# greysun/GraphEmbeddings

Hardware: AMD Instinct MI355X
Metric: scored triples/sec/GPU (d=200) (higher is better)
Workload: dtype f32

## Files before the change

### graphembeddings_amd/csrc/ge_prep.h

```cpp
#pragma once
#include "ge_common.h"

namespace ge {

constexpr int kSlotDirect = -2;
constexpr int kPrepThreads = 1024;
constexpr int kPrepWaves = kPrepThreads / kWave;
constexpr int kItemCap = 16;
constexpr int64_t kSub = 4096;
constexpr int kMaxRadix = 256;
constexpr unsigned long long kInvalidKey = ~0ull;

__host__ __device__ inline int64_t step_row(int64_t first_row, int64_t T, int64_t B, int64_t s) {
  int64_t first = first_row % T;
  if (first + B > T) first = 0;
  const int64_t n0 = (T - first) / B;
  if (s < n0) return first + s * B;
  const int64_t per = T / B;
  return ((s - n0) % per) * B;
}

struct PrepLayout {
  int64_t B, negs, units, n_sub, S, P, off_slot, off_order, off_sub, sub_stride, off_items, off_islots, stride;
  int epu;
};
__host__ __device__ inline PrepLayout prep_layout(int64_t B, int64_t negs = 0) {
  PrepLayout L;
  L.B = B;
  L.negs = negs;
  L.epu = negs > 0 ? 3 : 4;
  L.units = negs > 0 ? (1 + negs) * B : B;
  L.n_sub = (L.units + kSub - 1) / kSub;
  const int64_t s = L.units < kSub ? L.units : kSub;
  const int64_t gran = negs > 0 ? 1024 : 256;
  L.S = (s + gran - 1) / gran * gran;
  L.P = L.epu * L.S;
  L.off_slot = 3 * B;
  L.off_order = (negs == 0 && L.n_sub > 1) ? 9 * B : -1;
  L.off_sub = negs > 0 ? (3 * negs * B + 63) / 64 * 64 : ((L.off_order >= 0 ? 10 : 9) * B + 63) / 64 * 64;
  L.off_items = 64;
  L.off_islots = 64 + 2 * L.P;
  L.sub_stride = 64 + 2 * L.P + kItemCap * L.P;
  L.stride = L.off_sub + L.n_sub * L.sub_stride;
  return L;
}

struct TileGeom {
  int P, n_sub;
  int64_t stride;
  int64_t off_slot;
  int64_t off_sub, sub_stride;
  int off_items, off_islots;
};
inline TileGeom geom_of(const PrepLayout& L) {
  return TileGeom{(int)L.P, (int)L.n_sub, L.stride, L.off_slot, L.off_sub, L.sub_stride, (int)L.off_items, (int)L.off_islots};
}
inline TileGeom geom_plain(int P, int n_sub) {
  const int64_t sub = 64 + 2 * (int64_t)P + kItemCap * (int64_t)P;
  return TileGeom{P, n_sub, n_sub * sub, -1, 0, sub, 64, 64 + 2 * P};
}

struct ShardOut {
  int32_t R;
  int64_t B;
  int32_t* pos_src;
  int32_t* neg_src;
  int32_t* req_row;
  const int32_t* tile_heads;
  int32_t peer;
};

struct SortBits { int n_pass, bits; };
inline SortBits sort_bits_for(int64_t N) {
  int nbits = 1;
  while (((int64_t)1 << nbits) <= N) ++nbits;
  SortBits s;
  s.n_pass = (nbits + 7) / 8;
  s.bits = (nbits + s.n_pass - 1) / s.n_pass;
  if (s.bits < 6) s.bits = 6;
  return s;
}

__device__ __forceinline__ int wave_incl_add(int v, int lane) {
#pragma unroll
  for (int o = 1; o < kWave; o <<= 1) { const int t = __shfl_up(v, o, kWave); if (lane >= o) v += t; }
  return v;
}
__device__ __forceinline__ int wave_incl_max(int v, int lane) {
#pragma unroll
  for (int o = 1; o < kWave; o <<= 1) { const int t = __shfl_up(v, o, kWave); if (lane >= o) v = max(v, t); }
  return v;
}

struct StepSource {
  const int32_t* pos; int64_t B; const int32_t* id_to_type; int64_t N; const int64_t* type_offsets;
  int32_t n_types; const int32_t* type_ids; uint64_t seed, step; int32_t padded_size, mode, negs;
};

__device__ __forceinline__ void unit_keys(const StepSource& S, int64_t j, bool batch_heads, int32_t* __restrict__ neg,
                                          unsigned long long (&k)[4]) {
  if (S.negs > 0) {
    const int64_t B = S.B;
    const int64_t i = j < B ? j : (j - B) % B;
    int32_t t3[3] = {S.pos[3 * i], S.pos[3 * i + 1], S.pos[3 * i + 2]};
    if (j >= B) {
      const int64_t kk = (j - B) / B;
      const uint64_t stepk = S.step * (uint64_t)S.negs + (uint64_t)kk;
      const bool heads_k = (S.mode == GE_CORRUPT_BATCH_COIN) ? batch_coin_heads(S.seed, stepk) : false;
      int col;
      const int32_t repl = corrupt_one(t3, i, heads_k, S.id_to_type, S.N, S.type_offsets, S.n_types, S.type_ids, S.seed,
                                       stepk, S.padded_size, S.mode, col);
      t3[col] = repl;
      int32_t* o = neg + 3 * (kk * B + i);
      o[0] = t3[0]; o[1] = t3[1]; o[2] = t3[2];
    }
    const bool bad = t3[0] < 0 || t3[1] < 0 || t3[2] < 0 || t3[0] >= S.N || t3[1] >= S.N || t3[2] >= S.N;
#pragma unroll
    for (int X = 0; X < 3; ++X)
      k[X] = bad ? kInvalidKey : (((unsigned long long)(uint32_t)t3[X] << 32) | (uint32_t)(3 * j + X));
    k[3] = kInvalidKey;
    return;
  }
  const int64_t i = j;
  int32_t p[3] = {S.pos[3 * i], S.pos[3 * i + 1], S.pos[3 * i + 2]};
  int col;
  const int32_t repl = corrupt_one(p, i, batch_heads, S.id_to_type, S.N, S.type_offsets, S.n_types, S.type_ids, S.seed,
                                   S.step, S.padded_size, S.mode, col);
  int32_t n[3] = {p[0], p[1], p[2]};
  n[col] = repl;
  neg[3 * i] = n[0]; neg[3 * i + 1] = n[1]; neg[3 * i + 2] = n[2];
  const bool bad = p[0] < 0 || p[1] < 0 || p[2] < 0 || p[0] >= S.N || p[1] >= S.N || p[2] >= S.N || repl < 0 || repl >= S.N;
#pragma unroll
  for (int X = 0; X < 3; ++X)
    k[X] = bad ? kInvalidKey : (((unsigned long long)(uint32_t)p[X] << 32) | (uint32_t)(6 * i + X));
  k[3] = (bad || repl == p[col]) ? kInvalidKey : (((unsigned long long)(uint32_t)repl << 32) | (uint32_t)(6 * i + 3 + col));
}

}
```

### graphembeddings_amd/csrc/ge_train.hip

```cpp
#include "ge_prep.h"
#include "ge_launch.h"
#include <cmath>

namespace ge {

__global__ __launch_bounds__(kPrepThreads) void train_prepare_kernel(
    const int32_t* __restrict__ triples, int64_t T, int64_t first_row, int64_t B, int64_t s0,
    const int32_t* __restrict__ id_to_type, int64_t N, const int64_t* __restrict__ type_offsets,
    int32_t n_types, const int32_t* __restrict__ type_ids, uint64_t seed, uint64_t global_step0,
    int32_t padded_size, int32_t mode, int direct, int n_pass, int bits, int negs, int32_t* __restrict__ prep) {
  extern __shared__ __attribute__((aligned(16))) unsigned long long keys[];
  const PrepLayout L = prep_layout(B, negs);
  const int P = (int)L.P, R = P / kPrepThreads;
  unsigned* hist = reinterpret_cast<unsigned*>(keys + P);
  int* wtot = reinterpret_cast<int*>(hist + kPrepWaves * kMaxRadix);
  const int tid = threadIdx.x, lane = tid & (kWave - 1), wave = tid >> 6;
  const int sub = blockIdx.y;
  const int64_t s = s0 + blockIdx.x;
  const int32_t* pos = triples + 3 * step_row(first_row, T, B, s);
  int32_t* rec = prep + (int64_t)blockIdx.x * L.stride;
  int32_t* neg = rec;
  int32_t* slot_item = rec + L.off_slot;
  int32_t* subrec = rec + L.off_sub + sub * L.sub_stride;
  int32_t* items = subrec + L.off_items;
  int32_t* islots = subrec + L.off_islots;
  const int64_t i0 = (int64_t)sub * kSub;
  const int S = (int)((L.units - i0) < kSub ? (L.units - i0) : kSub);
  const uint64_t step = global_step0 + (uint64_t)s;
  const bool batch_heads = (mode == GE_CORRUPT_BATCH_COIN) ? batch_coin_heads(seed, step) : false;
  constexpr unsigned long long kInvalid = ~0ull;

  if (direct)
    for (int i = tid; i < 6 * S; i += kPrepThreads) slot_item[6 * i0 + i] = -1;

  {
    const StepSource src{pos, B, id_to_type, N, type_offsets, n_types, type_ids, seed, step, padded_size, mode, negs};
    for (int il = tid; il < (int)L.S; il += kPrepThreads) {
      unsigned long long k4[4] = {kInvalid, kInvalid, kInvalid, kInvalid};
      if (il < S) unit_keys(src, i0 + il, batch_heads, neg, k4);
      if (negs > 0) {
#pragma unroll
        for (int X = 0; X < 3; ++X) keys[3 * il + X] = k4[X];
      } else {
#pragma unroll
        for (int X = 0; X < 4; ++X) keys[4 * il + X] = k4[X];
      }
    }
  }
  __syncthreads();

  const int radix = 1 << bits;
  const unsigned dmask = (unsigned)radix - 1u;
  const int seg = kWave * R;
  for (int pass = 0; pass < n_pass; ++pass) {
    const int shift = 32 + pass * bits;
    for (int i = tid; i < radix * kPrepWaves; i += kPrepThreads) hist[i] = 0;
    __syncthreads();
    unsigned long long k[16];
    unsigned off[16];
#pragma unroll
    for (int r = 0; r < 16; ++r) {
      if (r < R) {
        k[r] = keys[wave * seg + r * kWave + lane];
        const unsigned dg = (unsigned)(k[r] >> shift) & dmask;
        unsigned long long peers = ~0ull;
        for (int b = 0; b < bits; ++b) {
          const bool bit = (dg >> b) & 1u;
          const unsigned long long bal = __ballot(bit);
          peers &= bit ? bal : ~bal;
        }
        const unsigned rank = (unsigned)__popcll(peers & ((1ull << lane) - 1ull));
        const unsigned cnt = (unsigned)__popcll(peers);
        unsigned* hp = hist + dg * kPrepWaves + wave;
        const unsigned base = *hp;
        __builtin_amdgcn_wave_barrier();
        if (rank == 0) *hp = base + cnt;
        __builtin_amdgcn_wave_barrier();
        off[r] = base + rank;
      }
    }
    __syncthreads();
    {
      const int q = radix * kPrepWaves / kPrepThreads;
      unsigned loc[4];
      int sum = 0;
      for (int u = 0; u < q; ++u) { loc[u] = hist[tid * q + u]; sum += (int)loc[u]; }
      const int incl = wave_incl_add(sum, lane);
      if (lane == kWave - 1) wtot[wave] = incl;
      __syncthreads();
      int run = incl - sum;
      for (int w = 0; w < wave; ++w) run += wtot[w];
      for (int u = 0; u < q; ++u) { hist[tid * q + u] = (unsigned)run; run += (int)loc[u]; }
    }
    __syncthreads();
#pragma unroll
    for (int r = 0; r < 16; ++r) {
      if (r < R) {
        const unsigned dg = (unsigned)(k[r] >> shift) & dmask;
        keys[hist[dg * kPrepWaves + wave] + off[r]] = k[r];
      }
    }
    __syncthreads();
  }

  auto key_at = [&](int i) -> unsigned long long { return (i >= 0 && i < P) ? keys[i] : kInvalid; };
  int rs_loc[16];
  {
    int carry = -1;
#pragma unroll
    for (int r = 0; r < 16; ++r) {
      if (r < R) {
        const int i = wave * seg + r * kWave + lane;
        const unsigned long long kk = keys[i], kp = key_at(i - 1);
        const bool head = kk != kInvalid && (i == 0 || (uint32_t)(kp >> 32) != (uint32_t)(kk >> 32));
        const int m = max(wave_incl_max(head ? i : -1, lane), carry);
        rs_loc[r] = m;
        carry = __shfl(m, kWave - 1, kWave);
      }
    }
    if (lane == 0) wtot[wave] = carry;
  }
  __syncthreads();
  int prev_max = -1;
  for (int w = 0; w < wave; ++w) prev_max = max(prev_max, wtot[w]);
  __syncthreads();
  unsigned start_mask = 0;
  int idx_loc[16];
  {
    int carry = 0;
#pragma unroll
    for (int r = 0; r < 16; ++r) {
      if (r < R) {
        const int i = wave * seg + r * kWave + lane;
        const unsigned long long kk = keys[i], kp = key_at(i - 1), kn = key_at(i + 1);
        const bool valid = kk != kInvalid;
        const uint32_t row = (uint32_t)(kk >> 32);
        const bool head = valid && (i == 0 || (uint32_t)(kp >> 32) != row);
        const bool sole = direct && head && !(kn != kInvalid && (uint32_t)(kn >> 32) == row);
        const int rs = max(rs_loc[r], prev_max);
        rs_loc[r] = rs;
        const bool start = valid && ((i - rs) % kItemCap) == 0 && !sole;
        if (start) start_mask |= 1u << r;
        if (sole) slot_item[(uint32_t)kk] = kSlotDirect;
        const int incl = wave_incl_add(start ? 1 : 0, lane) + carry;
        idx_loc[r] = incl - (start ? 1 : 0);
        carry = __shfl(incl, kWave - 1, kWave);
      }
    }
    if (lane == 0) wtot[wave] = carry;
  }
  __syncthreads();
  int prev_items = 0, total = 0;
  for (int w = 0; w < kPrepWaves; ++w) { if (w < wave) prev_items += wtot[w]; total += wtot[w]; }
  if (tid == 0) subrec[0] = total;
#pragma unroll
  for (int r = 0; r < 16; ++r) {
    if (r < R && ((start_mask >> r) & 1u)) {
      const int i = wave * seg + r * kWave + lane;
      const uint32_t row = (uint32_t)(keys[i] >> 32);
      const int idx = prev_items + idx_loc[r];
      int e = i + 1;
      while (e < P && (e - i) < kItemCap && keys[e] != kInvalid && (uint32_t)(keys[e] >> 32) == row) ++e;
      const bool more = (e < P && keys[e] != kInvalid && (uint32_t)(keys[e] >> 32) == row);
      const bool multi = (i != rs_loc[r]) || more;
      items[2 * idx] = (int32_t)row;
      items[2 * idx + 1] = (e - i) | (multi ? (1 << 30) : 0);
#pragma unroll
      for (int j = 0; j < kItemCap; ++j)
        islots[idx * kItemCap + j] = (i + j < e) ? (int32_t)(uint32_t)keys[i + j] : -1;
    }
  }
}

template <int NJ, bool COND, bool DET = false>
__global__ __launch_bounds__(kBlock) void apply_sorted_kernel(
    float* __restrict__ table, int d, const int32_t* __restrict__ sub0, int64_t sub_stride, int off_items,
    int off_islots, const int32_t* __restrict__ grad_idx, const float* grad_val, int split,
    float* __restrict__ out2) {
  const int lane = threadIdx.x & (kWave - 1);
  const int wave = (int)(((int64_t)blockIdx.x * blockDim.x + threadIdx.x) >> 6);
  const int nwaves = (int)(((int64_t)gridDim.x * blockDim.x) >> 6);
  const int32_t* subrec = sub0 + (int64_t)blockIdx.y * sub_stride;
  const int32_t* items = subrec + off_items;
  const int32_t* islots = subrec + off_islots;
  const int n_items = subrec[0];
  for (int w = wave; w < n_items; w += nwaves) {
    const int row = items[2 * w], cm = items[2 * w + 1];
    int slot_v = (lane < kItemCap) ? islots[w * kItemCap + lane] : -1;
    const int cnt = cm & 0x3FFFFFFF;
    const bool multi = (cm >> 30) & 1;
    const bool away = row >= split;
    float* dst = away ? out2 + (int64_t)(row - split) * d : table + (int64_t)row * d;
    float base[NJ];
#pragma unroll
    for (int j = 0; j < NJ; ++j) {
      const int c = lane + kWave * j;
      base[j] = (!multi && !away && c < d) ? dst[c] : 0.f;
    }
    const bool act_v = slot_v >= 0 && (!grad_idx || grad_idx[slot_v] >= 0);
    if (slot_v < 0) slot_v = 0;
    const unsigned long long live = __ballot(act_v);
    const bool park = DET && multi && !away;
    if (live == 0ull && !(away && !multi) && !park) continue;
    float acc[NJ];
#pragma unroll
    for (int j = 0; j < NJ; ++j) acc[j] = 0.f;
    for (int o = 0; o < cnt; o += 4) {
      int sl[4];
      bool on[4];
#pragma unroll
      for (int q = 0; q < 4; ++q) {
        const int src_lane = (o + q < cnt) ? (o + q) : o;
        sl[q] = __shfl(slot_v, src_lane, kWave);
        on[q] = (o + q < cnt) && ((live >> (o + q)) & 1ull);
      }
      float v[4][NJ];
#pragma unroll
      for (int q = 0; q < 4; ++q) {
        const float* src = grad_val + (int64_t)sl[q] * d;
#pragma unroll
        for (int j = 0; j < NJ; ++j) {
          const int c = lane + kWave * j;
          v[q][j] = (c < d && (!COND || on[q])) ? src[c] : 0.f;
        }
      }
#pragma unroll
      for (int q = 0; q < 4; ++q)
#pragma unroll
        for (int j = 0; j < NJ; ++j) acc[j] += on[q] ? v[q][j] : 0.f;
    }
    float* parked = const_cast<float*>(grad_val) + (int64_t)__shfl(slot_v, 0, kWave) * d;
#pragma unroll
    for (int j = 0; j < NJ; ++j) {
      const int c = lane + kWave * j;
      if (c < d) {
        if (park) parked[c] = acc[j];
        else if (multi) atomic_add_f32(dst + c, acc[j]);
        else dst[c] = base[j] + acc[j];
      }
    }
  }
}

constexpr int kHotBlock = 512;
template <int NJ>
__global__ __launch_bounds__(kHotBlock) void hot_rows_kernel(
    float* __restrict__ table, int d, const int32_t* __restrict__ sub0, int64_t sub_stride, int off_items, int off_islots,
    int n_sub, const float* __restrict__ grad_val) {
  constexpr int kScan = kWave;
  constexpr int kWv = kHotBlock / kWave;
  __shared__ int heads[kScan];
  __shared__ int n_heads;
  __shared__ float part[kWv - 1][NJ * kWave];
  const int t = threadIdx.x, lane = t & (kWave - 1), wv = t >> 6, tile = blockIdx.y;
  auto sub_of = [&](int tl) { return sub0 + (int64_t)tl * sub_stride; };
  const int32_t* subrec = sub_of(tile);
  const int n_items = subrec[0];
  for (int win = blockIdx.x; win * kScan < n_items; win += gridDim.x) {
  if (t == 0) n_heads = 0;
  __syncthreads();
  const int k = win * kScan + t;
  if (t < kScan && k < n_items) {
    const int32_t* items = subrec + off_items;
    const int row = items[2 * k], cm = items[2 * k + 1];
    if ((cm >> 30) & 1) {
      int prev_row = -1;
      if (k > 0) prev_row = items[2 * (k - 1)];
      else if (tile > 0) { const int32_t* ps = sub_of(tile - 1); const int pn = ps[0]; if (pn > 0) prev_row = ps[off_items + 2 * (pn - 1)]; }
      if (prev_row != row) heads[atomicAdd(&n_heads, 1)] = k;
    }
  }
  __syncthreads();
  const int nh = n_heads;
  auto item_at = [&](int k0, int r, int row, int& first_slot) -> bool {
    int idx = k0 + r, tl = tile;
    const int32_t* sr = subrec;
    int ni = n_items;
    while (idx >= ni) {
      idx -= ni; ++tl;
      if (tl >= n_sub) return false;
      sr = sub_of(tl); ni = sr[0];
    }
    first_slot = sr[off_islots + idx * kItemCap];
    return sr[off_items + 2 * idx] == row;
  };
  constexpr int kInFlight = NJ <= 4 ? 16 : 8;
  auto add_rows = [&](int fs, int n, float (&acc)[NJ]) {
    for (int o = 0; o < n; o += kInFlight) {
      float v[kInFlight][NJ];
#pragma unroll
      for (int q = 0; q < kInFlight; ++q)
        if (o + q < n) {
          const float* src = grad_val + (int64_t)__shfl(fs, o + q, kWave) * d;
#pragma unroll
          for (int j = 0; j < NJ; ++j) { const int c = lane + kWave * j; v[q][j] = src[c < d ? c : 0]; }
        }
#pragma unroll
      for (int q = 0; q < kInFlight; ++q)
        if (o + q < n) {
#pragma unroll
          for (int j = 0; j < NJ; ++j) acc[j] += v[q][j];
        }
    }
  };
  for (int h = wv; h < nh; h += kWv) {
    const int k0 = heads[h];
    const int row = (subrec + off_items)[2 * k0];
    int fs = 0;
    const bool mine = item_at(k0, lane, row, fs);
    const int n = __popcll(__ballot(mine));
    if (n == kWave) continue;
    float acc[NJ];
#pragma unroll
    for (int j = 0; j < NJ; ++j) acc[j] = 0.f;
    add_rows(fs, n, acc);
    float* dst = table + (int64_t)row * d;
#pragma unroll
    for (int j = 0; j < NJ; ++j) { const int c = lane + kWave * j; if (c < d) dst[c] = dst[c] + acc[j]; }
    if (lane == 0) heads[h] = -1;
  }
  __syncthreads();
  for (int h = 0; h < nh; ++h) {
    const int k0 = heads[h];
    if (k0 < 0) continue;
    const int row = (subrec + off_items)[2 * k0];
    float acc[NJ];
#pragma unroll
    for (int j = 0; j < NJ; ++j) acc[j] = 0.f;
    for (int r0 = wv; ; r0 += kWv * kWave) {
      int fs = 0;
      const bool mine = item_at(k0, r0 + kWv * lane, row, fs);
      const int n = __popcll(__ballot(mine));
      add_rows(fs, n, acc);
      if (n < kWave) break;
    }
    if (wv > 0) {
#pragma unroll
      for (int j = 0; j < NJ; ++j) part[wv - 1][j * kWave + lane] = acc[j];
    }
    __syncthreads();
    if (wv == 0) {
      float* dst = table + (int64_t)row * d;
#pragma unroll
      for (int j = 0; j < NJ; ++j) {
        const int c = lane + kWave * j;
        float tot = acc[j];
#pragma unroll
        for (int w2 = 0; w2 < kWv - 1; ++w2) tot += part[w2][j * kWave + lane];
        if (c < d) dst[c] = dst[c] + tot;
      }
    }
    __syncthreads();
  }
  __syncthreads();
  }
}

template <int VW, int NJ, bool DET = false>
__global__ __launch_bounds__(kBlock) void apply_rows_kernel(
    float* __restrict__ table, int d, const int32_t* __restrict__ sub0, int64_t sub_stride, int off_items,
    int off_islots, const int32_t* __restrict__ grad_idx, const float* grad_val, int split,
    float* __restrict__ out2) {
  typedef const __attribute__((address_space(4))) int32_t* kptr_t;
  constexpr int RG0 = 16 / (VW * NJ);
  constexpr int RG = RG0 > kItemCap ? kItemCap : (RG0 < 2 ? 2 : RG0);
  const int lane = threadIdx.x & (kWave - 1);
  const int wave = __builtin_amdgcn_readfirstlane((int)(((int64_t)blockIdx.x * blockDim.x + threadIdx.x) >> 6));
  const int nwaves = (int)(((int64_t)gridDim.x * blockDim.x) >> 6);
  const int32_t* subrec = sub0 + (int64_t)blockIdx.y * sub_stride;
  const kptr_t items = (kptr_t)(uintptr_t)(subrec + off_items);
  const int32_t* islots = subrec + off_islots;
  const int n_items = ((kptr_t)(uintptr_t)subrec)[0];
  int col[NJ];
  bool ok[NJ];
#pragma unroll
  for (int j = 0; j < NJ; ++j) { col[j] = VW * (lane + kWave * j); ok[j] = col[j] < d; if (!ok[j]) col[j] = 0; }
  for (int w = wave; w < n_items; w += nwaves) {
    const int row = items[2 * w], cm = items[2 * w + 1];
    int slot_v = (lane < kItemCap) ? islots[w * kItemCap + lane] : -1;
    const int cnt = cm & 0x3FFFFFFF;
    const bool multi = (cm >> 30) & 1;
    const bool away = row >= split;
    float* dst = away ? out2 + (int64_t)(row - split) * d : table + (int64_t)row * d;
    if (multi) {
      constexpr int ND = VW * NJ;
      const bool act_v = slot_v >= 0 && (!grad_idx || grad_idx[slot_v] >= 0);
      const unsigned long long lv = __ballot(act_v);
      const bool park = DET && !away;
      if (lv == 0ull && !park) continue;
      float a[ND];
#pragma unroll
      for (int j = 0; j < ND; ++j) a[j] = 0.f;
      for (int o = 0; o < cnt; o += 4) {
        float v[4][ND];
#pragma unroll
        for (int q = 0; q < 4; ++q)
          if (o + q < cnt && ((lv >> (o + q)) & 1ull)) {
            const float* src = grad_val + (int64_t)__builtin_amdgcn_readlane(slot_v, o + q) * d;
#pragma unroll
            for (int j = 0; j < ND; ++j) { const int c = lane + kWave * j; v[q][j] = src[c < d ? c : 0]; }
          }
#pragma unroll
        for (int q = 0; q < 4; ++q)
          if (o + q < cnt && ((lv >> (o + q)) & 1ull)) {
#pragma unroll
            for (int j = 0; j < ND; ++j) a[j] += v[q][j];
          }
      }
      float* parked = const_cast<float*>(grad_val) + (int64_t)__builtin_amdgcn_readlane(slot_v, 0) * d;
#pragma unroll
      for (int j = 0; j < ND; ++j) {
        const int c = lane + kWave * j;
        if (c < d) { if (park) parked[c] = a[j]; else atomic_add_f32(dst + c, a[j]); }
      }
      continue;
    }
    float base[NJ][VW];
#pragma unroll
    for (int j = 0; j < NJ; ++j) {
      if (!away) load_vec<VW>(dst + col[j], base[j]);
      else {
#pragma unroll
        for (int e = 0; e < VW; ++e) base[j][e] = 0.f;
      }
    }
    float acc[NJ][VW];
#pragma unroll
    for (int j = 0; j < NJ; ++j)
#pragma unroll
      for (int e = 0; e < VW; ++e) acc[j][e] = 0.f;
    unsigned long long live = 0ull;
    bool have_live = false;
    for (int o = 0; o < cnt; o += RG) {
      float v[RG][NJ][VW];
      if (!have_live) {
        const bool act_v = slot_v >= 0 && (!grad_idx || grad_idx[slot_v] >= 0);
        live = __ballot(act_v);
        have_live = true;
      }
#pragma unroll
      for (int q = 0; q < RG; ++q)
        if (o + q < cnt && ((live >> (o + q)) & 1ull)) {
          const int sl = __builtin_amdgcn_readlane(slot_v, o + q);
          const float* src = grad_val + (int64_t)sl * d;
#pragma unroll
          for (int j = 0; j < NJ; ++j) load_vec<VW>(src + col[j], v[q][j]);
        }
#pragma unroll
      for (int q = 0; q < RG; ++q)
        if (o + q < cnt && ((live >> (o + q)) & 1ull)) {
#pragma unroll
          for (int j = 0; j < NJ; ++j)
#pragma unroll
            for (int e = 0; e < VW; ++e) acc[j][e] += v[q][j][e];
        }
    }
    if (live == 0ull && !away) continue;
#pragma unroll
    for (int j = 0; j < NJ; ++j) {
      if (!ok[j]) continue;
      float o_[VW];
#pragma unroll
      for (int e = 0; e < VW; ++e) o_[e] = base[j][e] + acc[j][e];
      store_vec<VW>(dst + col[j], o_);
    }
  }
}

int apply_items_launch(float* table, int d, const TileGeom& G, const int32_t* step_rec, const int32_t* gidx,
                       const float* gval, int split, float* out2, hipStream_t st, hipEvent_t ev_start, hipEvent_t ev_stop,
                       int det) {
  const int grid = grid_for(G.P, kBlock / kWave);
  const int nj = (d + kWave - 1) / kWave;
  const dim3 g((unsigned)grid, (unsigned)G.n_sub);
  auto hot = [&]() -> int {
    const dim3 gh((unsigned)((G.P + kWave - 1) / kWave), (unsigned)G.n_sub);
#define LH(NJ) hipLaunchKernelGGL((hot_rows_kernel<NJ>), gh, dim3(kHotBlock), 0, st, table, d, step_rec + G.off_sub, G.sub_stride, G.off_items, G.off_islots, G.n_sub, gval)
    if (nj <= 1) LH(1); else if (nj <= 2) LH(2); else if (nj <= 4) LH(4); else if (nj <= 8) LH(8); else LH(16);
#undef LH
    return launch_status();
  };
  if (det && nj > 16) return GE_ENOTSUP;
#define LA(NJ)                                                                                                             \
  {                                                                                                                        \
    if (G.n_sub > 1) hipExtLaunchKernelGGL((apply_sorted_kernel<NJ, true>), g, dim3(kBlock), 0, st, ev_start, ev_stop, 0, table, d, step_rec + G.off_sub, G.sub_stride, G.off_items, G.off_islots, gidx, gval, split, out2); \
    else if (det) { hipExtLaunchKernelGGL((apply_sorted_kernel<NJ, false, true>), g, dim3(kBlock), 0, st, ev_start, ev_stop, 0, table, d, step_rec + G.off_sub, G.sub_stride, G.off_items, G.off_islots, gidx, gval, split, out2); return hot(); } \
    else hipExtLaunchKernelGGL((apply_sorted_kernel<NJ, false>), g, dim3(kBlock), 0, st, ev_start, ev_stop, 0, table, d, step_rec + G.off_sub, G.sub_stride, G.off_items, G.off_islots, gidx, gval, split, out2); \
  }
  if (gidx != nullptr || G.n_sub > 1) {
    auto al = [](const void* q, int a) { return q == nullptr || reinterpret_cast<uintptr_t>(q) % a == 0; };
    const int vw = (d % 4 == 0 && al(table, 16) && al(gval, 16) && al(out2, 16)) ? 4 : (d % 2 == 0 && al(table, 8) && al(gval, 8) && al(out2, 8)) ? 2 : 1;
    const int njr = (d / vw + kWave - 1) / kWave;
    const dim3 g((unsigned)(G.n_sub > 1 ? grid_for((G.P + 7) / 8, kBlock / kWave) : grid), (unsigned)G.n_sub);
#define LR(VW, NJ)                                                                                                       \
    {                                                                                                                    \
      if (det) {                                                                                                         \
        hipExtLaunchKernelGGL((apply_rows_kernel<VW, NJ, true>), g, dim3(kBlock), 0, st, ev_start, ev_stop, 0, table, d, \
                              step_rec + G.off_sub, G.sub_stride, G.off_items, G.off_islots, gidx, gval, split, out2);   \
        return hot();                                                                                                    \
      }                                                                                                                  \
      hipExtLaunchKernelGGL((apply_rows_kernel<VW, NJ>), g, dim3(kBlock), 0, st, ev_start, ev_stop, 0, table, d, \
                            step_rec + G.off_sub, G.sub_stride, G.off_items, G.off_islots, gidx, gval, split, out2);     \
      return launch_status();                                                                                            \
    }
    if (vw == 4) { if (njr <= 1) LR(4, 1) else if (njr <= 2) LR(4, 2) else if (njr <= 4) LR(4, 4) }
    else if (vw == 2) { if (njr <= 1) LR(2, 1) else if (njr <= 2) LR(2, 2) else if (njr <= 4) LR(2, 4) else if (njr <= 8) LR(2, 8) }
    else { if (njr <= 1) LR(1, 1) else if (njr <= 2) LR(1, 2) else if (njr <= 4) LR(1, 4) else if (njr <= 8) LR(1, 8) else if (njr <= 16) LR(1, 16) }
#undef LR
  }
  if (nj <= 1) LA(1) else if (nj <= 2) LA(2) else if (nj <= 4) LA(4) else if (nj <= 8) LA(8) else if (nj <= 16) LA(16)
  else return GE_ENOTSUP;
#undef LA
  return launch_status();
}

static int apply_sorted_launch(float* table, int d, const PrepLayout& L, const int32_t* step_rec, const int32_t* gidx,
                               const float* gval, hipStream_t st, hipEvent_t ev_start, hipEvent_t ev_stop, int det = 0) {
  return apply_items_launch(table, d, geom_of(L), step_rec, gidx, gval, 0x7FFFFFFF, nullptr, st, ev_start, ev_stop, det);
}

size_t hinge_ws_bytes(int64_t B, int32_t d) {
  return align_up(sizeof(int32_t) * 6 * (size_t)B, 256) + align_up(sizeof(float) * 6 * (size_t)B * (size_t)d, 256);
}

static bool train_fast_ok(int64_t B, int32_t d) { return B >= 1 && B <= (int64_t)1 << 24 && d <= 1024; }

static int64_t prep_chunk_steps(int64_t B, int64_t negs = 0) {
  const int64_t u = negs > 0 ? (1 + negs) * B : B;
  int64_t c = (32 * kSub) / (u < kSub ? kSub : u);
  const int64_t floor_steps = u <= 32768 ? 16 : u <= 4 * 65536 ? 8 : 2;
  return c < floor_steps ? floor_steps : c;
}

static size_t grad_region_bytes(int64_t B, int32_t d) {
  return align_up(sizeof(float) * 6 * (size_t)B * (size_t)d, 256);
}
static int grad_ring(int64_t B, int32_t d) {
  const size_t reg = grad_region_bytes(B, d);
  size_t r = ((size_t)64 << 20) / reg + 1;
  if (r < 2) r = 2;
  if (r > 16) r = 16;
  if (r < 4 && 4 * reg <= ((size_t)160 << 20)) r = 4;
  return (int)r;
}
static size_t train_grad_bytes(int64_t B, int32_t d) {
  return align_up(sizeof(int32_t) * 6 * (size_t)B, 256) + (size_t)grad_ring(B, d) * grad_region_bytes(B, d);
}
static size_t prep_chunk_bytes(int64_t B, int64_t negs = 0) {
  return align_up(sizeof(int32_t) * (size_t)prep_chunk_steps(B, negs) * (size_t)prep_layout(B, negs).stride, 256);
}
size_t train_ws_bytes(int64_t B, int32_t d) {
  if (!train_fast_ok(B, d)) return hinge_ws_bytes(B, d);
  return train_grad_bytes(B, d) + 2 * prep_chunk_bytes(B) + prep_big_scratch_bytes(B, 0, prep_chunk_steps(B));
}

static size_t prep_lds_bytes(const PrepLayout& L) {
  return sizeof(unsigned long long) * (size_t)L.P + sizeof(unsigned) * kPrepWaves * kMaxRadix + sizeof(int) * 32;
}

static int prepare_launch(const int32_t* triples, int64_t T, int64_t first_row, int64_t B, int64_t s0, int64_t n,
                          const int32_t* id_to_type, int64_t N, const int64_t* type_offsets, int32_t n_types,
                          const int32_t* type_ids, uint64_t seed, uint64_t global_step0, int32_t padded_size,
                          int32_t mode, int direct, int32_t* out, void* scratch, hipStream_t st, int negs = 0) {
  const PrepLayout L = prep_layout(B, negs);
  if (L.n_sub > 1)
    return prepare_big_launch(triples, T, first_row, B, s0, n, id_to_type, N, type_offsets, n_types, type_ids, seed,
                              global_step0, padded_size, mode, direct, out, scratch, st, negs);
  const SortBits sb = sort_bits_for(N);
  const int n_pass = sb.n_pass, bits = sb.bits;
  const size_t lds = prep_lds_bytes(L);
  hipError_t e = hipFuncSetAttribute(reinterpret_cast<const void*>(train_prepare_kernel),
                                     hipFuncAttributeMaxDynamicSharedMemorySize, 160 * 1024);
  if (e != hipSuccess) return (int)e;
  hipLaunchKernelGGL(train_prepare_kernel, dim3((unsigned)n, (unsigned)L.n_sub), dim3(kPrepThreads), lds, st, triples,
                     T, first_row, B, s0, id_to_type, N, type_offsets, n_types, type_ids, seed, global_step0,
                     padded_size, mode, direct, n_pass, bits, negs, out);
  return launch_status();
}

#define GE_HIP_TRY(expr) do { hipError_t e_ = (expr); if (e_ != hipSuccess) return (int)e_; } while (0)

struct Pipeline {
  int device = -1;
  hipStream_t side = nullptr;
  hipEvent_t prep_done[2] = {nullptr, nullptr};
  hipEvent_t buf_free[2] = {nullptr, nullptr};
  bool live = false;
  const int32_t* triples = nullptr; const int32_t* id_to_type = nullptr; const int64_t* type_offsets = nullptr;
  const int32_t* type_ids = nullptr; void* workspace = nullptr;
  int64_t T = 0, B = 0, N = 0, origin_row = 0, next_abs = 0, resident[2] = {-1, -1};
  uint64_t seed = 0, origin_gs = 0;
  int32_t n_types = 0, padded_size = 0, mode = 0, d = 0;
  int direct = 0, negs = 0;
};

int pipeline_create(void** out) {
  Pipeline* p = new Pipeline();
  hipError_t e = hipGetDevice(&p->device);
  if (e == hipSuccess) e = hipStreamCreateWithFlags(&p->side, hipStreamNonBlocking);
  for (int i = 0; i < 2 && e == hipSuccess; ++i) {
    e = hipEventCreateWithFlags(&p->prep_done[i], hipEventDisableTiming);
    if (e == hipSuccess) e = hipEventCreateWithFlags(&p->buf_free[i], hipEventDisableTiming);
  }
  if (e != hipSuccess) { delete p; return (int)e; }
  *out = p;
  return 0;
}
int pipeline_reset(void* h) {
  if (!h) return GE_EINVAL;
  static_cast<Pipeline*>(h)->live = false;
  return 0;
}
int pipeline_destroy(void* h) {
  if (!h) return GE_EINVAL;
  Pipeline* p = static_cast<Pipeline*>(h);
  if (p->side) { (void)hipStreamSynchronize(p->side); (void)hipStreamDestroy(p->side); }
  for (int i = 0; i < 2; ++i) {
    if (p->prep_done[i]) (void)hipEventDestroy(p->prep_done[i]);
    if (p->buf_free[i]) (void)hipEventDestroy(p->buf_free[i]);
  }
  delete p;
  return 0;
}

static inline int64_t norm_row(int64_t first_row, int64_t T, int64_t B) {
  int64_t f = first_row % T;
  if (f + B > T) f = 0;
  return f;
}

struct StepIdentity {
  const int32_t* triples; int64_t T, first_row, B; const int32_t* id_to_type; int64_t N;
  const int64_t* type_offsets; int32_t n_types; const int32_t* type_ids; uint64_t seed, global_step0;
  int32_t padded_size, mode, d; int direct, negs; void* workspace;
};

class PrepCursor {
 public:
  PrepCursor(const StepIdentity& id, Pipeline* handle, int32_t* prep_base, hipStream_t st)
      : id_(id), L_(prep_layout(id.B, id.negs)), K_(prep_chunk_steps(id.B, id.negs)),
        buf_ints_((int64_t)(prep_chunk_bytes(id.B, id.negs) / sizeof(int32_t))), base_(prep_base), st_(st),
        pipe_(handle ? handle : &local_), own_side_(handle != nullptr) {}

  int begin() {
    if (own_side_) {
      int dev = -1;
      GE_HIP_TRY(hipGetDevice(&dev));
      if (dev != pipe_->device) return GE_EINVAL;
      Pipeline* p = pipe_;
      const bool cont = p->live && p->triples == id_.triples && p->id_to_type == id_.id_to_type &&
                        p->type_offsets == id_.type_offsets && p->type_ids == id_.type_ids &&
                        p->workspace == id_.workspace && p->T == id_.T && p->B == id_.B && p->N == id_.N &&
                        p->seed == id_.seed && p->n_types == id_.n_types && p->padded_size == id_.padded_size &&
                        p->mode == id_.mode && p->d == id_.d && p->direct == id_.direct && p->negs == id_.negs &&
                        id_.global_step0 == p->origin_gs + (uint64_t)p->next_abs &&
                        norm_row(id_.first_row, id_.T, id_.B) == step_row(p->origin_row, id_.T, id_.B, p->next_abs);
      if (!cont) {
        p->live = true;
        p->triples = id_.triples; p->id_to_type = id_.id_to_type; p->type_offsets = id_.type_offsets;
        p->type_ids = id_.type_ids; p->workspace = id_.workspace; p->T = id_.T; p->B = id_.B; p->N = id_.N;
        p->seed = id_.seed; p->n_types = id_.n_types; p->padded_size = id_.padded_size; p->mode = id_.mode;
        p->d = id_.d; p->direct = id_.direct; p->negs = id_.negs;
        p->origin_row = norm_row(id_.first_row, id_.T, id_.B); p->origin_gs = id_.global_step0; p->next_abs = 0;
        p->resident[0] = p->resident[1] = -1;
      }
      base_abs_ = p->next_abs;
    } else {
      pipe_->origin_row = norm_row(id_.first_row, id_.T, id_.B);
      pipe_->origin_gs = id_.global_step0;
      pipe_->side = st_;
    }
    return 0;
  }

  int step(int64_t s, const int32_t** rec) {
    const int64_t abs_s = base_abs_ + s, chunk = abs_s / K_, in_chunk = abs_s % K_;
    if (s == 0 || in_chunk == 0) {
      int rc = ensure(chunk);
      if (rc) return rc;
      if (own_side_) {
        rc = ensure(chunk + 1);
        if (rc) return rc;
        GE_HIP_TRY(hipStreamWaitEvent(st_, pipe_->prep_done[chunk & 1], 0));
      }
    }
    *rec = base_ + (chunk & 1) * buf_ints_ + in_chunk * L_.stride;
    return 0;
  }

  int finish(int64_t n_steps, const int32_t** last_rec) {
    const int64_t la = base_abs_ + n_steps - 1;
    *last_rec = base_ + ((la / K_) & 1) * buf_ints_ + (la % K_) * L_.stride;
    if (own_side_) {
      GE_HIP_TRY(hipStreamWaitEvent(st_, pipe_->prep_done[((la / K_) + 1) & 1], 0));
      pipe_->next_abs = base_abs_ + n_steps;
    }
    return 0;
  }

  const PrepLayout& layout() const { return L_; }

 private:
  int ensure(int64_t c) {
    const int b = (int)(c & 1);
    if (pipe_->resident[b] == c) return 0;
    if (own_side_) {
      GE_HIP_TRY(hipEventRecord(pipe_->buf_free[b], st_));
      GE_HIP_TRY(hipStreamWaitEvent(pipe_->side, pipe_->buf_free[b], 0));
    }
    int rc = prepare_launch(id_.triples, id_.T, pipe_->origin_row, id_.B, c * K_, K_, id_.id_to_type, id_.N,
                            id_.type_offsets, id_.n_types, id_.type_ids, id_.seed, pipe_->origin_gs, id_.padded_size,
                            id_.mode, id_.direct, base_ + b * buf_ints_, base_ + 2 * buf_ints_, pipe_->side, id_.negs);
    if (rc) return rc;
    if (own_side_) GE_HIP_TRY(hipEventRecord(pipe_->prep_done[b], pipe_->side));
    pipe_->resident[b] = c;
    return 0;
  }

  StepIdentity id_;
  PrepLayout L_;
  int64_t K_, buf_ints_;
  int32_t* base_;
  hipStream_t st_;
  Pipeline local_;
  Pipeline* pipe_;
  bool own_side_;
  int64_t base_abs_ = 0;
};

int train_steps_run(float* table, int64_t N, int32_t d, const int32_t* triples, int64_t T, int64_t first_row,
                    int64_t B, int64_t n_steps, const int32_t* id_to_type, const int64_t* type_offsets,
                    int32_t n_types, const int32_t* type_ids, uint64_t seed, uint64_t global_step0,
                    int32_t padded_size, int32_t mode, float margin, float lr0, float decay_steps,
                    float decay_rate, float max_norm, int model, float* loss, int keep_all_losses,
                    int32_t* neg_ws, void* workspace, size_t workspace_bytes, void** ev_pairs, int ev_kernel,
                    void* pipe_handle, hipStream_t st) {
  if (n_steps <= 0) return 0;
  const int deterministic = (model & GE_STEP_DETERMINISTIC) ? 1 : 0;
  model &= ~GE_STEP_DETERMINISTIC;
  const bool transform = model == GE_MODEL_HOLE && !(d & 1);
  const bool spectral = transform || model == GE_MODEL_HOLE_SPECTRAL;
  const bool hole_direct = (model == GE_MODEL_HOLE && (d & 1)) || model == GE_MODEL_HOLE_DIRECT;
  if (transform) { int rc = hole_spectral_launch(table, N, d, 0, st); if (rc) return rc; }
  int32_t* gidx = reinterpret_cast<int32_t*>(workspace);
  float* gval0 = reinterpret_cast<float*>(reinterpret_cast<char*>(workspace) + align_up(sizeof(int32_t) * 6 * (size_t)B, 256));
  const bool fast = train_fast_ok(B, d) && workspace_bytes >= train_ws_bytes(B, d);
  const int ring = fast ? grad_ring(B, d) : 1;
  const size_t region_floats = grad_region_bytes(B, d) / sizeof(float);
  const int direct = hole_direct ? 0 : 1;
  const StepIdentity ident{triples, T, first_row, B, id_to_type, N, type_offsets, n_types, type_ids, seed, global_step0,
                           padded_size, mode, d, direct, 0, workspace};
  PrepCursor cur(ident, fast ? static_cast<Pipeline*>(pipe_handle) : nullptr,
                 reinterpret_cast<int32_t*>(reinterpret_cast<char*>(workspace) + train_grad_bytes(B, d)), st);
  const PrepLayout& L = cur.layout();
  if (fast) { int rc = cur.begin(); if (rc) return rc; }
  auto lr_at = [&](uint64_t gs) {
    return decay_steps > 0.f ? lr0 / (1.0f + decay_rate * ((float)gs / decay_steps)) : lr0;
  };
  for (int64_t s = 0; s < n_steps; ++s) {
    const uint64_t gs = global_step0 + (uint64_t)s;
    const float lr = lr_at(gs);
    const int32_t* pos = triples + 3 * step_row(first_row, T, B, s);
    float* loss_s = keep_all_losses ? loss + s * B : loss;
    hipEvent_t e0 = ev_pairs ? (hipEvent_t)ev_pairs[2 * s] : nullptr;
    hipEvent_t e1 = ev_pairs ? (hipEvent_t)ev_pairs[2 * s + 1] : nullptr;
    int rc;
    const int32_t* neg;
    const int32_t* step_rec = nullptr;
    if (e0 && ev_kernel == 0) (void)hipEventRecord(e0, st);
    if (fast) {
      rc = cur.step(s, &step_rec);
      if (rc) return rc;
      neg = step_rec;
    } else {
      rc = corrupt_batch_launch(pos, B, id_to_type, N, type_offsets, n_types, type_ids, seed, gs, padded_size,
                                mode, neg_ws, st);
      if (rc) return rc;
      neg = neg_ws;
    }
    if (e1 && ev_kernel == 0) (void)hipEventRecord(e1, st);
    float* gval = gval0 + (size_t)(gs % (uint64_t)ring) * region_floats;
    hipEvent_t g0 = ev_kernel == 1 ? e0 : nullptr, g1 = ev_kernel == 1 ? e1 : nullptr;
    hipEvent_t a0 = ev_kernel == 2 ? e0 : nullptr, a1 = ev_kernel == 2 ? e1 : nullptr;
    const bool dir = fast && direct;
    rc = hole_direct ? hole_hinge_grad_launch(table, N, d, pos, neg, B, margin, lr, max_norm, loss_s, gidx, gval, st, g0, g1)
                     : complex_hinge_grad_launch(table, N, d, pos, neg, B, margin, lr, max_norm, loss_s, gidx, gval, st, g0, g1,
                                                 dir ? step_rec + L.off_slot : nullptr, dir ? table : nullptr, spectral ? 1 : 0,
                                                 (fast && L.off_order >= 0) ? step_rec + L.off_order : nullptr);
    if (rc) return rc;
    if (fast) rc = apply_sorted_launch(table, d, L, step_rec, gidx, gval, st, a0, a1, deterministic);
    else rc = scatter_add_rows_launch(table, N, d, gidx, gval, 6 * B, st, a0, a1);
    if (rc) return rc;
  }
  if (fast) {
    const int32_t* last = nullptr;
    int rc = cur.finish(n_steps, &last);
    if (rc) return rc;
    GE_HIP_TRY(hipMemcpyAsync(neg_ws, last, sizeof(int32_t) * 3 * (size_t)B, hipMemcpyDeviceToDevice, st));
  }
  if (transform) { int rc = hole_spectral_launch(table, N, d, 1, st); if (rc) return rc; }
  return 0;
}

size_t train_logloss_ws_bytes(int64_t B, int32_t negs, int32_t d) {
  const size_t M = (size_t)(1 + negs) * (size_t)B;
  const size_t region = align_up(sizeof(float) * 3 * M * (size_t)d, 256);
  size_t ring = ((size_t)64 << 20) / region + 1;
  if (ring < 2) ring = 2;
  if (ring > 8) ring = 8;
  return 256 + align_up(sizeof(int32_t) * 3 * M, 256) + ring * region + 2 * prep_chunk_bytes(B, negs) +
         prep_big_scratch_bytes(B, negs, prep_chunk_steps(B, negs));
}

int train_logloss_run(float* table, int64_t N, int32_t d, const int32_t* triples, int64_t T, int64_t first_row,
                      int64_t B, int64_t n_steps, const int32_t* id_to_type, const int64_t* type_offsets,
                      int32_t n_types, const int32_t* type_ids, uint64_t seed, uint64_t global_step0,
                      int32_t padded_size, int32_t mode, int32_t negs, float l2, float lr0, float decay_steps,
                      float decay_rate, float max_norm, float* loss, int keep_all_losses, int32_t* neg_ws,
                      void* workspace, size_t workspace_bytes, void* pipe_handle, hipStream_t st) {
  if (n_steps <= 0) return 0;
  if (workspace_bytes < train_logloss_ws_bytes(B, negs, d)) return GE_ENOMEM;
  const size_t M = (size_t)(1 + negs) * (size_t)B;
  const size_t region = align_up(sizeof(float) * 3 * M * (size_t)d, 256);
  size_t ring = ((size_t)64 << 20) / region + 1;
  if (ring < 2) ring = 2;
  if (ring > 8) ring = 8;
  char* w = reinterpret_cast<char*>(workspace);
  float* sumsq = reinterpret_cast<float*>(w);
  int32_t* gidx = reinterpret_cast<int32_t*>(w + 256);
  char* gval0 = w + 256 + align_up(sizeof(int32_t) * 3 * M, 256);
  int32_t* prep_base = reinterpret_cast<int32_t*>(gval0 + ring * region);
  const StepIdentity ident{triples, T, first_row, B, id_to_type, N, type_offsets, n_types, type_ids, seed, global_step0,
                           padded_size, mode, d, 0, negs, workspace};
  PrepCursor cur(ident, static_cast<Pipeline*>(pipe_handle), prep_base, st);
  const PrepLayout& L = cur.layout();
  int rc = cur.begin();
  if (rc) return rc;
  double g = 1.0;
  auto materialise = [&]() -> int {
    if (g == 1.0) return 0;
    int r2 = table_scale_launch(table, N * (int64_t)d, (float)g, st);
    g = 1.0;
    return r2;
  };
  for (int64_t s = 0; s < n_steps; ++s) {
    const uint64_t gs = global_step0 + (uint64_t)s;
    const float lr = decay_steps > 0.f ? lr0 / (1.0f + decay_rate * ((float)gs / decay_steps)) : lr0;
    const int32_t* pos = triples + 3 * step_row(first_row, T, B, s);
    const int32_t* step_rec = nullptr;
    rc = cur.step(s, &step_rec);
    if (rc) return rc;
    const double f = 1.0 - (double)lr * (double)M * (double)l2;
    double g_new = g * f;
    if (g_new == 0.0 || std::fabs(g_new) < 9.1e-13 || std::fabs(g_new) > 1.1e12) {
      rc = materialise();
      if (rc) return rc;
      g_new = 1.0;
    }
    const bool want_loss = keep_all_losses || s == n_steps - 1;
    if (want_loss) { rc = table_sumsq_launch(table, N * (int64_t)d, sumsq, st); if (rc) return rc; }
    float* loss_s = keep_all_losses ? loss + s * (int64_t)M : loss;
    float* gval = reinterpret_cast<float*>(gval0 + (size_t)(gs % (uint64_t)ring) * region);
    const bool dense_now = (g_new == 1.0 && g * f != 1.0);
    const float neg_lr_eff = (float)(-(double)lr / (dense_now ? 1.0 : g_new));
    rc = complex_logloss_grad_launch(table, N, d, pos, nullptr, (int64_t)M, lr, max_norm, l2, want_loss ? sumsq : nullptr,
                                     loss_s, gidx, gval, st, step_rec, B, (float)g, neg_lr_eff, nullptr, nullptr);
    if (rc) return rc;
    if (dense_now) {
      rc = table_scale_launch(table, N * (int64_t)d, (float)f, st);
      if (rc) return rc;
    }
    rc = apply_sorted_launch(table, d, L, step_rec, gidx, gval, st, nullptr, nullptr);
    if (rc) return rc;
    g = g_new;
  }
  rc = materialise();
  if (rc) return rc;
  const int32_t* last = nullptr;
  rc = cur.finish(n_steps, &last);
  if (rc) return rc;
  GE_HIP_TRY(hipMemcpyAsync(neg_ws, last, sizeof(int32_t) * 3 * (size_t)negs * (size_t)B, hipMemcpyDeviceToDevice, st));
  return 0;
}

size_t train_prepare_bytes(int64_t B, int64_t n_steps) {
  return align_up(sizeof(int32_t) * (size_t)n_steps * (size_t)prep_layout(B).stride, 256) + prep_big_scratch_bytes(B, 0, n_steps);
}
int train_prepare_run(const int32_t* triples, int64_t T, int64_t first_row, int64_t B, int64_t n_steps,
                      const int32_t* id_to_type, int64_t N, const int64_t* type_offsets, int32_t n_types,
                      const int32_t* type_ids, uint64_t seed, uint64_t global_step0, int32_t padded_size,
                      int32_t mode, int direct, int32_t* out, hipStream_t st) {
  if (n_steps == 0) return 0;
  void* scratch = reinterpret_cast<char*>(out) + align_up(sizeof(int32_t) * (size_t)n_steps * (size_t)prep_layout(B).stride, 256);
  return prepare_launch(triples, T, norm_row(first_row, T, B), B, 0, n_steps, id_to_type, N, type_offsets, n_types,
                        type_ids, seed, global_step0, padded_size, mode, direct ? 1 : 0, out, scratch, st);
}

void train_prepared_layout(int64_t B, int64_t* out) {
  const PrepLayout L = prep_layout(B);
  out[0] = L.stride; out[1] = L.n_sub; out[2] = L.S; out[3] = L.off_slot; out[4] = L.off_sub;
  out[5] = L.sub_stride; out[6] = L.off_items; out[7] = L.off_islots;
}

}
```

Baseline: 542.8 million.

## Add single-tile apply kernel with hot-row directory for multi-item rows

The prepare kernel now also writes a directory of 'hot' rows, meaning rows whose gradient items span several item records, with the first item index and count for each. A new single-launch apply kernel gives dedicated workgroups to these hot rows, reducing their items across waves through shared memory and writing each row once. The remaining workgroups handle single-item rows with a grid-stride loop. This is meant to remove the cost of the split or atomic handling of multi-item rows in the generic path when there is one subtile, at the price of extra prep work, a larger prep record and possible load imbalance.

```diff
diff --git a/graphembeddings_amd/csrc/ge_prep.h b/graphembeddings_amd/csrc/ge_prep.h
--- a/graphembeddings_amd/csrc/ge_prep.h
+++ b/graphembeddings_amd/csrc/ge_prep.h
@@ -20,8 +20,9 @@
   return ((s - n0) % per) * B;
 }
 
+__host__ __device__ inline int64_t hot_dir_words(int64_t P) { return (1 + 2 * (P / (kItemCap + 1) + 1) + 63) / 64 * 64; }
 struct PrepLayout {
-  int64_t B, negs, units, n_sub, S, P, off_slot, off_order, off_sub, sub_stride, off_items, off_islots, stride;
+  int64_t B, negs, units, n_sub, S, P, off_slot, off_order, off_sub, sub_stride, off_items, off_islots, off_hot, stride;
   int epu;
 };
 __host__ __device__ inline PrepLayout prep_layout(int64_t B, int64_t negs = 0) {
@@ -40,7 +41,8 @@
   L.off_sub = negs > 0 ? (3 * negs * B + 63) / 64 * 64 : ((L.off_order >= 0 ? 10 : 9) * B + 63) / 64 * 64;
   L.off_items = 64;
   L.off_islots = 64 + 2 * L.P;
-  L.sub_stride = 64 + 2 * L.P + kItemCap * L.P;
+  L.off_hot = L.off_islots + kItemCap * L.P;
+  L.sub_stride = L.off_hot + hot_dir_words(L.P);
   L.stride = L.off_sub + L.n_sub * L.sub_stride;
   return L;
 }
diff --git a/graphembeddings_amd/csrc/ge_train.hip b/graphembeddings_amd/csrc/ge_train.hip
--- a/graphembeddings_amd/csrc/ge_train.hip
+++ b/graphembeddings_amd/csrc/ge_train.hip
@@ -153,6 +153,7 @@
   int prev_items = 0, total = 0;
   for (int w = 0; w < kPrepWaves; ++w) { if (w < wave) prev_items += wtot[w]; total += wtot[w]; }
   if (tid == 0) subrec[0] = total;
+  unsigned last_mask = 0;
 #pragma unroll
   for (int r = 0; r < 16; ++r) {
     if (r < R && ((start_mask >> r) & 1u)) {
@@ -165,9 +166,40 @@
       const bool multi = (i != rs_loc[r]) || more;
       items[2 * idx] = (int32_t)row;
       items[2 * idx + 1] = (e - i) | (multi ? (1 << 30) : 0);
+      if (multi && !more) last_mask |= 1u << r;
 #pragma unroll
       for (int j = 0; j < kItemCap; ++j)
         islots[idx * kItemCap + j] = (i + j < e) ? (int32_t)(uint32_t)keys[i + j] : -1;
+    }
+  }
+  __syncthreads();
+  int hot_loc[16];
+  {
+    int carry = 0;
+#pragma unroll
+    for (int r = 0; r < 16; ++r) {
+      if (r < R) {
+        const int f = (int)((last_mask >> r) & 1u);
+        const int incl = wave_incl_add(f, lane) + carry;
+        hot_loc[r] = incl - f;
+        carry = __shfl(incl, kWave - 1, kWave);
+      }
+    }
+    if (lane == 0) wtot[wave] = carry;
+  }
+  __syncthreads();
+  int prev_hot = 0, total_hot = 0;
+  for (int w = 0; w < kPrepWaves; ++w) { if (w < wave) prev_hot += wtot[w]; total_hot += wtot[w]; }
+  int32_t* hot = subrec + L.off_hot;
+  if (tid == 0) hot[0] = total_hot;
+#pragma unroll
+  for (int r = 0; r < 16; ++r) {
+    if (r < R && ((last_mask >> r) & 1u)) {
+      const int i = wave * seg + r * kWave + lane;
+      const int before = (i - rs_loc[r]) / kItemCap;
+      const int h = prev_hot + hot_loc[r];
+      hot[1 + 2 * h] = prev_items + idx_loc[r] - before;
+      hot[2 + 2 * h] = before + 1;
     }
   }
 }
@@ -467,6 +499,214 @@
   }
 }
 
+constexpr int kTileBlock = 512;
+#ifndef GE_EXP_TILE_ROWS
+#define GE_EXP_TILE_ROWS 16
+#endif
+template <int VW, int NJ>
+__global__ __launch_bounds__(kTileBlock) void apply_rows_kernel_one_tile(
+    float* __restrict__ table, int d, const int32_t* __restrict__ subrec, int off_items, int off_islots, int off_hot,
+    const int32_t* __restrict__ grad_idx, const float* __restrict__ grad_val, int hot_wgs) {
+  typedef const __attribute__((address_space(4))) int32_t* kptr_t;
+  constexpr int ND = VW * NJ;
+  constexpr int RG0 = 64 / ND;
+  constexpr int RG = RG0 > GE_EXP_TILE_ROWS ? GE_EXP_TILE_ROWS : (RG0 < 2 ? 2 : RG0);
+  constexpr int kWv = kTileBlock / kWave;
+  constexpr int kPart = (128 / ND) < kWv ? kWv : (128 / ND);
+  __shared__ float part[kPart][ND * kWave];
+  const int lane = threadIdx.x & (kWave - 1);
+  const int wv = __builtin_amdgcn_readfirstlane((int)(threadIdx.x >> 6));
+  const kptr_t items = (kptr_t)(uintptr_t)(subrec + off_items);
+  const int32_t* islots = subrec + off_islots;
+  int col[NJ];
+  bool ok[NJ];
+#pragma unroll
+  for (int j = 0; j < NJ; ++j) { col[j] = VW * (lane + kWave * j); ok[j] = col[j] < d; if (!ok[j]) col[j] = 0; }
+  auto add_item = [&](int slot_v, int cnt, unsigned long long live, float (&acc)[NJ][VW]) {
+    for (int o = 0; o < cnt; o += RG) {
+      float v[RG][NJ][VW];
+#pragma unroll
+      for (int q = 0; q < RG; ++q)
+        if (o + q < cnt && ((live >> (o + q)) & 1ull)) {
+          const float* src = grad_val + (int64_t)__builtin_amdgcn_readlane(slot_v, o + q) * d;
+#pragma unroll
+          for (int j = 0; j < NJ; ++j) load_vec<VW>(src + col[j], v[q][j]);
+        }
+#pragma unroll
+      for (int q = 0; q < RG; ++q)
+        if (o + q < cnt && ((live >> (o + q)) & 1ull)) {
+#pragma unroll
+          for (int j = 0; j < NJ; ++j)
+#pragma unroll
+            for (int e = 0; e < VW; ++e) acc[j][e] += v[q][j][e];
+        }
+    }
+  };
+
+  if ((int)blockIdx.x < hot_wgs) {
+    const kptr_t hot = (kptr_t)(uintptr_t)(subrec + off_hot);
+    int h = blockIdx.x;
+    int first = hot[1 + 2 * h], n = hot[2 + 2 * h];
+    const int n_hot = hot[0];
+    while (h < n_hot) {
+      const int row = items[2 * first];
+      float* dst = table + (int64_t)row * d;
+      float base[NJ][VW], tot[NJ][VW];
+#pragma unroll
+      for (int j = 0; j < NJ; ++j) {
+        if (wv == 0) load_vec<VW>(dst + col[j], base[j]);
+#pragma unroll
+        for (int e = 0; e < VW; ++e) tot[j][e] = 0.f;
+      }
+      auto item_sum = [&](int it, float (&p)[NJ][VW]) {
+        const int w = first + it;
+        const int cnt = items[2 * w + 1] & 0x3FFFFFFF;
+        const int slot_v = (lane < kItemCap) ? islots[w * kItemCap + lane] : -1;
+        const bool act_v = slot_v >= 0 && grad_idx[slot_v] >= 0;
+        const unsigned long long live = __ballot(act_v);
+#pragma unroll
+        for (int j = 0; j < NJ; ++j)
+#pragma unroll
+          for (int e = 0; e < VW; ++e) p[j][e] = 0.f;
+        add_item(slot_v, cnt, live, p);
+      };
+      if (n < kWave) {
+        for (int b0 = 0; b0 < n; b0 += kPart) {
+          const int b1 = min(n, b0 + kPart);
+          for (int it = b0 + wv; it < b1; it += kWv) {
+            float p[NJ][VW];
+            item_sum(it, p);
+#pragma unroll
+            for (int j = 0; j < NJ; ++j)
+#pragma unroll
+              for (int e = 0; e < VW; ++e) part[it - b0][(j * VW + e) * kWave + lane] = p[j][e];
+          }
+          __syncthreads();
+          if (wv == 0)
+            for (int it = 0; it < b1 - b0; ++it) {
+#pragma unroll
+              for (int j = 0; j < NJ; ++j)
+#pragma unroll
+                for (int e = 0; e < VW; ++e) tot[j][e] += part[it][(j * VW + e) * kWave + lane];
+            }
+          __syncthreads();
+        }
+      } else {
+        for (int it = wv; it < n; it += kWv) {
+          float p[NJ][VW];
+          item_sum(it, p);
+#pragma unroll
+          for (int j = 0; j < NJ; ++j)
+#pragma unroll
+            for (int e = 0; e < VW; ++e) tot[j][e] += p[j][e];
+        }
+        if (wv > 0) {
+#pragma unroll
+          for (int j = 0; j < NJ; ++j)
+#pragma unroll
+            for (int e = 0; e < VW; ++e) part[wv - 1][(j * VW + e) * kWave + lane] = tot[j][e];
+        }
+        __syncthreads();
+        if (wv == 0) {
+#pragma unroll
+          for (int w2 = 0; w2 < kWv - 1; ++w2)
+#pragma unroll
+            for (int j = 0; j < NJ; ++j)
+#pragma unroll
+              for (int e = 0; e < VW; ++e) tot[j][e] += part[w2][(j * VW + e) * kWave + lane];
+        }
+        __syncthreads();
+      }
+      if (wv == 0) {
+#pragma unroll
+        for (int j = 0; j < NJ; ++j) {
+          if (!ok[j]) continue;
+          float o_[VW];
+#pragma unroll
+          for (int e = 0; e < VW; ++e) o_[e] = base[j][e] + tot[j][e];
+          store_vec<VW>(dst + col[j], o_);
+        }
+      }
+      h += hot_wgs;
+      if (h >= n_hot) break;
+      first = hot[1 + 2 * h]; n = hot[2 + 2 * h];
+    }
+    return;
+  }
+
+  const int nwaves = (int)((gridDim.x - hot_wgs) * kWv);
+  int w = __builtin_amdgcn_readfirstlane((int)(blockIdx.x - hot_wgs) * kWv + wv);
+#ifdef GE_EXP_TILE_NITEMS_FIRST
+  const int n_items = ((kptr_t)(uintptr_t)subrec)[0];
+  if (w >= n_items) return;
+#endif
+  int row = items[2 * w], cm = items[2 * w + 1];
+  int slot_v = (lane < kItemCap) ? islots[w * kItemCap + lane] : -1;
+#ifndef GE_EXP_TILE_NITEMS_FIRST
+  const int n_items = ((kptr_t)(uintptr_t)subrec)[0];
+#endif
+  while (w < n_items) {
+    if (!((cm >> 30) & 1)) {
+      const int cnt = cm & 0x3FFFFFFF;
+      float* dst = table + (int64_t)row * d;
+      float base[NJ][VW], acc[NJ][VW];
+#pragma unroll
+      for (int j = 0; j < NJ; ++j) {
+        load_vec<VW>(dst + col[j], base[j]);
+#pragma unroll
+        for (int e = 0; e < VW; ++e) acc[j][e] = 0.f;
+      }
+      const bool act_v = slot_v >= 0 && grad_idx[slot_v] >= 0;
+      const unsigned long long live = __ballot(act_v);
+      add_item(slot_v, cnt, live, acc);
+      if (live != 0ull) {
+#pragma unroll
+        for (int j = 0; j < NJ; ++j) {
+          if (!ok[j]) continue;
+          float o_[VW];
+#pragma unroll
+          for (int e = 0; e < VW; ++e) o_[e] = base[j][e] + acc[j][e];
+          store_vec<VW>(dst + col[j], o_);
+        }
+      }
+    }
+    w += nwaves;
+    if (w >= n_items) break;
+    row = items[2 * w]; cm = items[2 * w + 1];
+    slot_v = (lane < kItemCap) ? islots[w * kItemCap + lane] : -1;
+  }
+}
+
+static int apply_one_tile_launch(float* table, int d, const PrepLayout& L, const int32_t* step_rec, const int32_t* gidx,
+                                 const float* gval, hipStream_t st, hipEvent_t ev_start, hipEvent_t ev_stop) {
+  auto al = [](const void* q, int a) { return reinterpret_cast<uintptr_t>(q) % a == 0; };
+  const int vw = (d % 4 == 0 && al(table, 16) && al(gval, 16)) ? 4 : (d % 2 == 0 && al(table, 8) && al(gval, 8)) ? 2 : 1;
+  const int njr = (d / vw + kWave - 1) / kWave;
+  constexpr int kWv = kTileBlock / kWave;
+  const int hot_cap = (int)(L.P / (kItemCap + 1));
+#ifndef GE_EXP_TILE_HOT_WGS
+#define GE_EXP_TILE_HOT_WGS 160
+#endif
+  const int hot_wgs = hot_cap < GE_EXP_TILE_HOT_WGS ? hot_cap : GE_EXP_TILE_HOT_WGS;
+#ifndef GE_EXP_TILE_KEYS_PER_WAVE
+#define GE_EXP_TILE_KEYS_PER_WAVE 4
+#endif
+  const int item_wgs = grid_for((L.P + GE_EXP_TILE_KEYS_PER_WAVE - 1) / GE_EXP_TILE_KEYS_PER_WAVE, kWv);
+  const dim3 g((unsigned)(hot_wgs + item_wgs));
+  const int32_t* subrec = step_rec + L.off_sub;
+#define LT(VW, NJ)                                                                                                         \
+  {                                                                                                                        \
+    hipExtLaunchKernelGGL((apply_rows_kernel_one_tile<VW, NJ>), g, dim3(kTileBlock), 0, st, ev_start, ev_stop, 0, table,  \
+                          d, subrec, (int)L.off_items, (int)L.off_islots, (int)L.off_hot, gidx, gval, hot_wgs);            \
+    return launch_status();                                                                                                \
+  }
+  if (vw == 4) { if (njr <= 1) LT(4, 1) else if (njr <= 2) LT(4, 2) else if (njr <= 4) LT(4, 4) }
+  else if (vw == 2) { if (njr <= 1) LT(2, 1) else if (njr <= 2) LT(2, 2) else if (njr <= 4) LT(2, 4) else if (njr <= 8) LT(2, 8) }
+  else { if (njr <= 1) LT(1, 1) else if (njr <= 2) LT(1, 2) else if (njr <= 4) LT(1, 4) else if (njr <= 8) LT(1, 8) else if (njr <= 16) LT(1, 16) }
+#undef LT
+  return GE_ENOTSUP;
+}
+
 int apply_items_launch(float* table, int d, const TileGeom& G, const int32_t* step_rec, const int32_t* gidx,
                        const float* gval, int split, float* out2, hipStream_t st, hipEvent_t ev_start, hipEvent_t ev_stop,
                        int det) {
@@ -516,6 +756,10 @@
 
 static int apply_sorted_launch(float* table, int d, const PrepLayout& L, const int32_t* step_rec, const int32_t* gidx,
                                const float* gval, hipStream_t st, hipEvent_t ev_start, hipEvent_t ev_stop, int det = 0) {
+#ifndef GE_EXP_TILE_OFF
+  if (L.n_sub == 1 && gidx != nullptr && d <= 16 * kWave)
+    return apply_one_tile_launch(table, d, L, step_rec, gidx, gval, st, ev_start, ev_stop);
+#endif
   return apply_items_launch(table, d, geom_of(L), step_rec, gidx, gval, 0x7FFFFFFF, nullptr, st, ev_start, ev_stop, det);
 }
 
```

Measured after the change: 435.7 million. -19.7%, worse.
